# i2nico/MDAnalysis-MPI

Hardware: AMD Instinct MI355X
Metric: atom-frames/sec (RMSF) + achieved HBM GB/s fraction (higher is better)
Workload: dtype f64

## Files before the change

include/rmsf_hip.h:

```cpp
#ifndef RMSF_HIP_H
#define RMSF_HIP_H

#include <stddef.h>
#include <stdint.h>

#ifdef __cplusplus
extern "C" {
#endif

#define RMSF_ABI_VERSION 3

#define RMSF_OK 0
#define RMSF_EINVAL (-1)
#define RMSF_EHIP (-2)
#define RMSF_ENOMEM (-3)
#define RMSF_EEMPTY (-4)

#define RMSF_MODE_WELFORD 0
#define RMSF_MODE_SUM 1

#define RMSF_XFORM_DOUBLES 16
#define RMSF_MAX_SPLIT_FRAMES 4096
#define RMSF_PAIR_NEWTON 0
#define RMSF_PAIR_JACOBI 1
// ... 168 lines not shown
                                     double *d_ref, double *d_refinfo,
                                     void *stream);
int rmsf_reference_sums_sequential(int64_t n_sel, double mass_total,
                                   const double *d_ref, double *d_refinfo,
                                   void *stream);
int rmsf_superpose_sequential(const float *d_xyz, int64_t frame_stride,
                              int64_t n_frames, int64_t n_sel,
                              const int32_t *d_sel, const double *d_masses,
                              double mass_total, const double *d_ref,
                              const double *d_refinfo, double *d_xform,
                              void *stream);
int rmsf_frame_com_sequential(const float *d_xyz, int64_t frame_stride,
                              int64_t n_frames, int64_t n_sel,
                              const int32_t *d_sel, const double *d_masses,
                              double mass_total, double *d_xform, void *stream);
int rmsf_superpose_sequential_from_com(const float *d_xyz, int64_t frame_stride,
                                       int64_t n_frames, int64_t n_sel,
                                       const int32_t *d_sel, const double *d_ref,
                                       const double *d_refinfo, double *d_xform,
                                       void *stream);
int rmsf_inner_product_sequential(const float *d_xyz, int64_t frame_stride,
                                  int64_t n_frames, int64_t n_sel,
                                  const int32_t *d_sel, const double *d_ref,
                                  double *d_xform, void *stream);
int rmsf_superpose_sequential_qcp(int64_t n_frames, int64_t n_sel,
                                  const double *d_refinfo, double *d_xform,
                                  void *stream);
int rmsf_accumulate_sequential(const float *d_xyz, int64_t frame_stride,
                               int64_t n_frames, int64_t n_sel,
                               const int32_t *d_sel, const double *d_xform,
                               const double *d_refinfo, int mode, int64_t k0,
                               double *d_acc0, double *d_acc1, void *d_work,
                               size_t work_bytes, void *stream);

int rmsf_finalize(const double *d_m2, int64_t n_sel, int64_t n_frames,
                  double *d_rmsf, void *stream);

size_t rmsf_covariance_workspace_bytes(int64_t n_sel, int64_t n_frames);
int rmsf_covariance_accumulate(const float *d_xyz, int64_t frame_stride,
                               int64_t n_frames, int64_t n_sel,
                               const int32_t *d_sel, const double *d_xform,
                               const double *d_refinfo, const double *d_shift,
                               double *d_cov, int64_t ld, double *d_t1,
                               void *d_work, size_t work_bytes, void *stream);
int rmsf_covariance_finish(double *d_cov, int64_t ld, const double *d_t1,
                           int64_t n_coord, int64_t n_frames, void *stream);

size_t rmsf_pca_project_workspace_bytes(int64_t n_frames, int64_t n_sel,
                                        int64_t n_comp);
int rmsf_pca_project(const float *d_xyz, int64_t frame_stride,
                     int64_t n_frames, int64_t n_sel, const int32_t *d_sel,
                     const double *d_xform, const double *d_refinfo,
                     const double *d_mean, const double *d_comp, int64_t ldc,
                     int64_t n_comp, double *d_out, int64_t ldo, void *d_work,
                     size_t work_bytes, void *stream);

size_t rmsf_pca_backproject_workspace_bytes(int64_t n_frames, int64_t n_sel,
                                            int64_t n_cols);
int rmsf_pca_backproject(const float *d_xyz, int64_t frame_stride,
                         int64_t n_frames, int64_t n_sel, const int32_t *d_sel,
                         const double *d_xform, const double *d_refinfo,
                         const double *d_mean, const double *d_p, int64_t ldp,
                         int64_t n_cols, double *d_y, int64_t ldy,
                         int accumulate, void *d_work, size_t work_bytes,
                         void *stream);

// ... 234 lines not shown
```

mdanalysis-mpi_amd/csrc/rmsf_kernels.hip:

```cpp
#include <hip/hip_runtime.h>

#include <algorithm>
#include <cmath>
#include <cstdint>
#include <cstring>
#include <mutex>
#include <string>
#include <type_traits>
#include <unordered_map>
#include <vector>

#include "rmsf_hip.h"
#include "rmsf_device.h"

#define RMSF_EXPORT __attribute__((visibility("default")))
#ifndef RMSF_SHIFTED_SUMS
#define RMSF_SHIFTED_SUMS 1
#endif

namespace {

thread_local std::string g_err;

int fail(int code, const std::string &msg) {
// ... 291 lines not shown
  hdr[8] = p.S;
  hdr[9] = p.cw;
}

template <int U>
__global__ __launch_bounds__(kBlock) void k_welford_flat_sk(const float *__restrict__ xyz, int64_t stride4,
                                                            SkPlan pl, int64_t *__restrict__ hdr,
                                                            double *__restrict__ parts0,
                                                            double *__restrict__ parts1) {
  const int b = sk_range(pl, blockIdx.x);
  if (blockIdx.x == 0 && threadIdx.x == 0) sk_write_header(hdr, pl);
  int64_t lo = sk_lo(pl, b);
  const int64_t hi = sk_lo(pl, b + 1);
  int64_t slot = (int64_t)b * pl.P;
  while (lo < hi) {
    int64_t c, f0;
    const int len = (int)sk_seg_len(pl, lo, hi, &c, &f0);
    const int64_t i4 = c * kBlock + threadIdx.x;
    if (i4 < pl.lanes) {
      double m[4], q[4];
      wel_flat_run<U>(reinterpret_cast<const f32x4 *>(xyz) + f0 * stride4 + i4, stride4, len, m, q);
      const int64_t o = slot * (kBlock * 4) + 4 * threadIdx.x;
      store4(parts0 + o, parts1 + o, m, q);
    }
    lo += len;
    ++slot;
  }
}

struct SeqCoef {
  double c, r;
};

__global__ __launch_bounds__(kBlock) void k_seq_coef(int64_t k0, int64_t nf, SeqCoef *__restrict__ out) {
  const int64_t f = (int64_t)blockIdx.x * kBlock + threadIdx.x;
  if (f >= nf) return;
  const double k = (double)(k0 + f), k1 = k + 1.0;
  double r = __builtin_amdgcn_rcp(k1);
  double e = __builtin_fma(-k1, r, 1.0);
  r = __builtin_fma(r, e, r);
  e = __builtin_fma(-k1, r, 1.0);
  r = __builtin_fma(r, e, r);
  out[f] = SeqCoef{k / k1, r};
}

__device__ __forceinline__ double seq_div(double num, double k1, double r) {
  const double q0 = num * r;
  const double q = __builtin_fma(__builtin_fma(-k1, q0, num), r, q0);
  return (num == 0.0 || __builtin_isinf(num)) ? num : q;
}

template <int U, bool GATHER>
__global__ __launch_bounds__(kBlock) void k_welford_seq(const float *__restrict__ xyz, int64_t fstride, int64_t nf,
                                                        int64_t n_coord, const int32_t *__restrict__ sel,
                                                        int64_t k0, const SeqCoef *__restrict__ coef,
                                                        double *__restrict__ mean, double *__restrict__ ss) {
  const int64_t j = (int64_t)blockIdx.x * kBlock + threadIdx.x;
  if (j >= n_coord) return;
  double m = k0 > 0 ? mean[j] : 0.0, q = k0 > 0 ? ss[j] : 0.0;
  const float *__restrict__ p = xyz + (GATHER ? 3 * (int64_t)sel[j / 3] + j % 3 : j);
  auto step = [&](float v, const SeqCoef cf, double k, double k1) {
    const double x = (double)v;
    const double d = x - m;
    q = q + cf.c * (d * d);
    m = seq_div(k * m + x, k1, cf.r);
  };
  auto load = [&](float (&v)[U], SeqCoef (&c)[U], int64_t f) {
#pragma unroll
    for (int u = 0; u < U; ++u) {
      v[u] = __builtin_nontemporal_load(p + (f + u) * fstride);
      c[u] = coef[f + u];
    }
  };
  auto step_fast = [&](float v, const SeqCoef cf, double k, double k1) {
    const double x = (double)v;
    const double d = x - m;
// ... 440 lines not shown
                                                          int64_t n_sel, const int32_t *__restrict__ sel,
                                                          const double *__restrict__ ref, double *__restrict__ xform) {
  RMSF_SEQ_SLICE;
  const int64_t f = blockIdx.x;
  const int j = blockIdx.y;
  const float *__restrict__ fr = xyz + f * fstride;
  const double *t = xform + f * kXform;
  auto row = [&](int64_t a) -> int64_t { return 3 * (GATHER ? (int64_t)sel[a] : a); };
  double s;
  if (j < 9) {
    const int ax = j / 3, rb = j % 3;
    const double cx = t[9 + ax];
    s = RMSF_SEQ_SUM(
        n_sel, [&](int64_t a) { return SeqF1D{fr[row(a) + ax], ref[3 * a + rb]}; },
        [&](const SeqF1D &v, int64_t) { return ((double)v.x - cx) * v.d; });
  } else {
    const double c0 = t[9], c1 = t[10], c2 = t[11];
    s = RMSF_SEQ_SUM(
        n_sel,
        [&](int64_t a) {
          const float *p = fr + row(a);
          return SeqF3{p[0], p[1], p[2]};
        },
        [&](const SeqF3 &v, int64_t) {
          const double x1 = (double)v.x - c0, y1 = (double)v.y - c1, z1 = (double)v.z - c2;
          return x1 * x1 + y1 * y1 + z1 * z1;
        });
  }
  if (threadIdx.x == 0) xform[f * kXform + (j < 9 ? j : 13)] = s;
}
#undef RMSF_SEQ_SUM
#undef RMSF_SEQ_SLICE

__global__ __launch_bounds__(64) void k_seq_qcp(int64_t n_frames, int64_t n_sel, const double *__restrict__ refinfo,
                                                double *__restrict__ xform) {
  const int64_t f = (int64_t)blockIdx.x * 64 + threadIdx.x;
  if (f >= n_frames) return;
  double *t = xform + f * kXform;
  double A[9];
#pragma unroll
  for (int j = 0; j < 9; ++j) A[j] = t[j];
  const double E0 = (t[13] + refinfo[6]) * 0.5;
  double rot[9], rmsd;
  qcp_solve(A, E0, (double)n_sel, rot, &rmsd);
#pragma unroll
  for (int j = 0; j < 9; ++j) t[j] = rot[j];
  t[12] = rmsd;
  t[13] = t[14] = t[15] = 0.0;
}

template <int MODE, bool ALIGN, bool GATHER, int U>
__global__ __launch_bounds__(kBlock) void k_accum_seq(const float *__restrict__ xyz, int64_t fstride, int64_t nf,
                                                      int64_t n_sel, const int32_t *__restrict__ sel,
                                                      const double *__restrict__ xform,
                                                      const double *__restrict__ refinfo, int64_t k0,
                                                      const SeqCoef *__restrict__ coef, double *__restrict__ acc0,
                                                      double *__restrict__ acc1) {
  const int64_t a = (int64_t)blockIdx.x * kBlock + threadIdx.x;
  if (a >= n_sel) return;
  const double rc0 = ALIGN ? refinfo[0] : 0.0, rc1 = ALIGN ? refinfo[1] : 0.0, rc2 = ALIGN ? refinfo[2] : 0.0;
  double m[3], q[3] = {0.0, 0.0, 0.0};
#pragma unroll
  for (int c = 0; c < 3; ++c) {
    m[c] = k0 > 0 ? acc0[3 * a + c] : 0.0;
    if (MODE == RMSF_MODE_WELFORD && k0 > 0) q[c] = acc1[3 * a + c];
  }
  const float *__restrict__ p = xyz + 3 * (GATHER ? (int64_t)sel[a] : a);
  auto consume = [&](float x, float y, float z, int64_t f, double k) {
    if (ALIGN) apply_xform(x, y, z, xform + f * kXform, rc0, rc1, rc2);
    const float v[3] = {x, y, z};
    if (MODE == RMSF_MODE_SUM) {
#pragma unroll
      for (int c = 0; c < 3; ++c) m[c] = m[c] + (double)v[c];
    } else {
      const SeqCoef cf = coef[f];
#pragma unroll
      for (int c = 0; c < 3; ++c) {
        const double xx = (double)v[c];
        const double d = xx - m[c];
        q[c] = q[c] + cf.c * (d * d);
        m[c] = seq_div(k * m[c] + xx, k + 1.0, cf.r);
      }
    }
  };
  int64_t f = 0;
  double kb = (double)k0;
  for (; f + U <= nf; f += U) {
    float v[U][3];
#pragma unroll
    for (int u = 0; u < U; ++u) {
      const float *r = p + (f + u) * fstride;
#pragma unroll
      for (int c = 0; c < 3; ++c) v[u][c] = __builtin_nontemporal_load(r + c);
    }
#pragma unroll
    for (int u = 0; u < U; ++u, kb += 1.0) consume(v[u][0], v[u][1], v[u][2], f + u, kb);
  }
  for (; f < nf; ++f, kb += 1.0) {
    const float *r = p + f * fstride;
    consume(r[0], r[1], r[2], f, kb);
  }
#pragma unroll
  for (int c = 0; c < 3; ++c) {
    acc0[3 * a + c] = m[c];
    if (MODE == RMSF_MODE_WELFORD) acc1[3 * a + c] = q[c];
  }
}

template <int MODE, bool ALIGN, bool GATHER, int U, bool PLANES = false>
__global__ __launch_bounds__(kBlock) void k_accum_atoms_sk(const float *__restrict__ xyz, int64_t fstride,
                                                           const int32_t *__restrict__ sel,
                                                           const double *__restrict__ xform,
                                                           const double *__restrict__ refinfo, SkPlan pl,
                                                           int64_t *__restrict__ hdr, double *__restrict__ parts0,
                                                           double *__restrict__ parts1, int64_t ps = 0) {
  const int b = sk_range(pl, blockIdx.x);
  if (blockIdx.x == 0 && threadIdx.x == 0) sk_write_header(hdr, pl);
  const double rc0 = ALIGN ? refinfo[0] : 0.0, rc1 = ALIGN ? refinfo[1] : 0.0, rc2 = ALIGN ? refinfo[2] : 0.0;
  int64_t lo = uni64(sk_lo(pl, b));
  const int64_t hi = uni64(sk_lo(pl, b + 1));
  int64_t slot = (int64_t)b * pl.P;
  while (lo < hi) {
    int64_t c, f0;
    const int len = __builtin_amdgcn_readfirstlane((int)sk_seg_len(pl, lo, hi, &c, &f0));
    c = uni64(c);
    f0 = uni64(f0);
    const int64_t a = c * kBlock + threadIdx.x;
    if (a < pl.lanes) {
      const int64_t off = (PLANES ? 1 : 3) * (GATHER ? (int64_t)sel[a] : a);
      double m[3], q[3];
      accum_atoms_run<MODE, ALIGN, U, PLANES>(xyz + f0 * fstride + off, fstride, len,
                                              ALIGN ? xform + f0 * kXform : nullptr, rc0, rc1, rc2, m, q, ps);
      const int64_t o = slot * (kBlock * 3) + 3 * threadIdx.x;
      store3<MODE>(parts0 + o, parts1 + o, m, q);
    }
    lo += len;
    ++slot;
  }
}
// ... 2024 lines not shown
    if (d_sel) SEQIP(true, false);
    else SEQIP(false, false);
  }
#undef SEQIP
  return after_launch("k_seq_ip");
}

RMSF_EXPORT int rmsf_superpose_sequential_qcp(int64_t n_frames, int64_t n_sel, const double *d_refinfo,
                                              double *d_xform, void *stream) {
  if (!d_refinfo || !d_xform || n_sel < 1 || n_frames < 0)
    return fail(RMSF_EINVAL, "rmsf_superpose_sequential_qcp: bad arguments");
  if (n_frames == 0) return RMSF_OK;
  const unsigned fb = (unsigned)((n_frames + 63) / 64);
  hipLaunchKernelGGL(k_seq_qcp, dim3(fb), dim3(64), 0, S(stream), n_frames, n_sel, d_refinfo, d_xform);
  return after_launch("k_seq_qcp");
}

RMSF_EXPORT int rmsf_superpose_sequential_from_com(const float *d_xyz, int64_t fstride, int64_t n_frames,
                                                   int64_t n_sel, const int32_t *d_sel, const double *d_ref,
                                                   const double *d_refinfo, double *d_xform, void *stream) {
  if (!d_xyz || !d_ref || !d_refinfo || !d_xform || n_sel < 1 || n_frames < 0 || fstride < (d_sel ? 3 : 3 * n_sel))
    return fail(RMSF_EINVAL, "rmsf_superpose_sequential_from_com: bad arguments");
  if (int rc = rmsf_inner_product_sequential(d_xyz, fstride, n_frames, n_sel, d_sel, d_ref, d_xform, stream))
    return rc;
  return rmsf_superpose_sequential_qcp(n_frames, n_sel, d_refinfo, d_xform, stream);
}

RMSF_EXPORT int rmsf_superpose_sequential(const float *d_xyz, int64_t fstride, int64_t n_frames, int64_t n_sel,
                                          const int32_t *d_sel, const double *d_masses, double mass_total,
                                          const double *d_ref, const double *d_refinfo, double *d_xform,
                                          void *stream) {
  if (!d_xyz || !d_ref || !d_refinfo || !d_xform || n_sel < 1 || n_frames < 0 || fstride < (d_sel ? 3 : 3 * n_sel))
    return fail(RMSF_EINVAL, "rmsf_superpose_sequential: bad arguments");
  if (int rc = rmsf_frame_com_sequential(d_xyz, fstride, n_frames, n_sel, d_sel, d_masses, mass_total, d_xform,
                                         stream))
    return rc;
  return rmsf_superpose_sequential_from_com(d_xyz, fstride, n_frames, n_sel, d_sel, d_ref, d_refinfo, d_xform,
                                            stream);
}

RMSF_EXPORT int rmsf_accumulate_sequential(const float *d_xyz, int64_t fstride, int64_t n_frames, int64_t n_sel,
                                           const int32_t *d_sel, const double *d_xform, const double *d_refinfo,
                                           int mode, int64_t k0, double *d_acc0, double *d_acc1, void *d_work,
                                           size_t work_bytes, void *stream) {
  const bool wel = mode == RMSF_MODE_WELFORD;
  if ((mode != RMSF_MODE_WELFORD && mode != RMSF_MODE_SUM) || !d_xyz || !d_acc0 || (wel && (!d_acc1 || !d_work)) ||
      n_sel < 1 || n_frames < 0 || k0 < 0 || k0 + n_frames > (int64_t(1) << 53) ||
      fstride < (d_sel ? 3 : 3 * n_sel) || (d_xform != nullptr) != (d_refinfo != nullptr))
    return fail(RMSF_EINVAL, "rmsf_accumulate_sequential: bad arguments");
  if (n_frames == 0) return RMSF_OK;
  hipStream_t s = S(stream);
  const SeqCoef *coef = nullptr;
  if (wel) {
    if (work_bytes < rmsf_welford_sequential_workspace_bytes(n_frames))
      return fail(RMSF_EINVAL, "rmsf_accumulate_sequential: workspace too small");
    hipLaunchKernelGGL(k_seq_coef, dim3(grid1(n_frames)), dim3(kBlock), 0, s, k0, n_frames,
                       static_cast<SeqCoef *>(d_work));
    if (int rc = after_launch("k_seq_coef")) return rc;
    coef = static_cast<const SeqCoef *>(d_work);
  }
  const bool al = d_xform != nullptr, g = d_sel != nullptr;
  const dim3 grid((unsigned)grid1(n_sel));
#define SEQACC(MO, A, G)                                                                                    \
  hipLaunchKernelGGL((k_accum_seq<MO, A, G, 4>), grid, dim3(kBlock), 0, s, d_xyz, fstride, n_frames, n_sel, d_sel, \
                     d_xform, d_refinfo, k0, coef, d_acc0, d_acc1)
  auto launch = [&](auto MOc) {
    constexpr int MO = decltype(MOc)::value;
    if (al && g) SEQACC(MO, true, true);
    else if (al) SEQACC(MO, true, false);
    else if (g) SEQACC(MO, false, true);
    else SEQACC(MO, false, false);
  };
#undef SEQACC
  if (wel) launch(std::integral_constant<int, RMSF_MODE_WELFORD>{});
  else launch(std::integral_constant<int, RMSF_MODE_SUM>{});
  return after_launch("k_accum_seq");
}

RMSF_EXPORT int rmsf_finalize(const double *d_m2, int64_t n_sel, int64_t n_frames, double *d_rmsf, void *stream) {
  if (!d_m2 || !d_rmsf || n_sel < 1) return fail(RMSF_EINVAL, "rmsf_finalize: bad arguments");
  if (n_frames < 1) return fail(RMSF_EEMPTY, "rmsf_finalize: no frames");
  hipLaunchKernelGGL(k_finalize, dim3(grid1(n_sel)), dim3(kBlock), 0, S(stream), d_m2, n_sel, (double)n_frames,
                     d_rmsf);
  return after_launch("k_finalize");
}

RMSF_EXPORT int rmsf_qcp_batch(const double *d_A, const double *d_E0, const double *d_N, int64_t n, double *d_rot,
                               double *d_rmsd, void *stream) {
  if (!d_A || !d_E0 || !d_N || !d_rot || !d_rmsd || n < 0) return fail(RMSF_EINVAL, "rmsf_qcp_batch: bad arguments");
  if (n == 0) return RMSF_OK;
  hipLaunchKernelGGL(k_qcp_batch, dim3(grid1(n)), dim3(kBlock), 0, S(stream), d_A, d_E0, d_N, n, d_rot, d_rmsd);
  return after_launch("k_qcp_batch");
}

RMSF_EXPORT int rmsf_calc_rmsd_rotational_matrix(const double *h_ref, const double *h_conf, int64_t N, double *h_rot,
                                                 const double *h_weights, double *rmsd_out) {
  if (!h_ref || !h_conf || !h_rot || N < 1) return fail(RMSF_EINVAL, "CalcRMSDRotationalMatrix: bad arguments");
  const size_t cb = (size_t)N * 3 * sizeof(double);
  double *d = nullptr;
  const size_t total = 2 * cb + (size_t)N * sizeof(double) + 32 * sizeof(double);
  HIP_TRY(hipMalloc(&d, total));
  double *dref = d, *dconf = d + 3 * N, *dw = d + 6 * N, *dio = d + 7 * N;
  int rc = RMSF_OK;
  do {
    hipError_t e;
    if ((e = hipMemcpy(dref, h_ref, cb, hipMemcpyHostToDevice)) != hipSuccess) { rc = hip_fail("memcpy", e); break; }
    if ((e = hipMemcpy(dconf, h_conf, cb, hipMemcpyHostToDevice)) != hipSuccess) { rc = hip_fail("memcpy", e); break; }
    if (h_weights && (e = hipMemcpy(dw, h_weights, N * sizeof(double), hipMemcpyHostToDevice)) != hipSuccess) {
      rc = hip_fail("memcpy", e);
// ... 83 lines not shown
```

mdanalysis-mpi_amd/rmsf_amd/_lib.py:

```python
from __future__ import annotations

import ctypes
import os
from ctypes import POINTER, c_char_p, c_double, c_int, c_int32, c_int64, c_size_t, c_uint64, c_void_p

_HERE = os.path.dirname(os.path.abspath(__file__))
LIB_PATH = os.path.normpath(os.path.join(_HERE, "..", "lib", "librmsf_hip.so"))

RMSF_OK = 0
RMSF_EINVAL = -1
RMSF_EHIP = -2
RMSF_ENOMEM = -3
RMSF_EEMPTY = -4
RMSF_MODE_WELFORD = 0
RMSF_MODE_SUM = 1
RMSF_XFORM_DOUBLES = 16
RMSF_MAX_SPLIT_FRAMES = 4096
RMSF_REFINFO_DOUBLES = 2064
ABI_VERSION = 3
RMSF_PAIR_NEWTON = 0
RMSF_PAIR_JACOBI = 1
RMSF_PAIR_ZERO = 2


class RmsfError(RuntimeError):

    def __init__(self, code: int, func: str, msg: str):
        super().__init__(f"{func} failed with status {code}: {msg}")
        self.code = code


class RmsfEmptyError(RmsfError, ZeroDivisionError):
    """No frames to reduce.  Subclasses ZeroDivisionError because RMSF.py:39
    raises exactly that when two empty partials are merged."""


P = c_void_p
SIGNATURES = {
    "rmsf_abi_version": (c_int, []),
    "rmsf_last_error": (c_char_p, []),
    "rmsf_device_count": (c_int, [POINTER(c_int)]),
    "rmsf_set_device": (c_int, [c_int]),
    "rmsf_malloc": (c_int, [POINTER(c_void_p), c_size_t]),
    "rmsf_free": (c_int, [P]),
    "rmsf_memcpy_h2d": (c_int, [P, P, c_size_t, P]),
    "rmsf_memcpy_d2h": (c_int, [P, P, c_size_t, P]),
    "rmsf_memcpy2d_d2d": (c_int, [P, c_size_t, P, c_size_t, c_size_t, c_size_t, P]),
    "rmsf_stream_synchronize": (c_int, [P]),
# ... 2 lines not shown
    "rmsf_reference_setup_mean": (c_int, [P, c_double, c_int64, P, P, P, P, P]),
    "rmsf_fold_balanced_finalize": (c_int, [P, c_int64, c_int64, P, P, c_int64, P, P]),
    "rmsf_superpose_workspace_bytes": (c_size_t, [c_int64, c_int64]),
    "rmsf_superpose": (c_int, [P, c_int64, c_int64, c_int64, P, P, P, P, P, P, c_size_t, P]),
    "rmsf_superpose_planes": (c_int, [P, c_int64, c_int64, c_int64, c_int64, P, P, P, P, P, P, c_size_t, P]),
    "rmsf_superpose_compact": (c_int, [P, c_int64, c_int64, c_int64, P, P, P, P, P, P, c_size_t, P, c_int64, P]),
    "rmsf_accumulate_splits": (c_int, [c_int64, c_int64, c_int]),
    "rmsf_accumulate": (c_int, [P, c_int64, c_int64, c_int64, P, P, P, c_int, c_int, P, P, P]),
    "rmsf_split_count": (c_int64, [c_int64, c_int, c_int]),
    "rmsf_accumulate_balanced_workspace_bytes": (c_size_t, [c_int64, c_int64, c_int]),
    "rmsf_accumulate_balanced": (c_int, [P, c_int64, c_int64, c_int64, P, P, P, c_int, c_int, P, c_size_t, P]),
    "rmsf_fold_balanced": (c_int, [P, c_int64, c_int, c_int64, P, P, P]),
    "rmsf_accumulate_balanced_planes": (c_int, [P, c_int64, c_int64, c_int64, c_int64, P, P, P, c_int, c_int, P,
                                                c_size_t, P]),
    "rmsf_chan_merge": (c_int, [P, P, P, c_int, c_int64, P, P, P]),
    "rmsf_chan_reduce_steps": (c_int, [c_int, c_int, P, P, c_int]),
    "rmsf_chan_reduce": (c_int, [P, P, P, c_int, c_int64, c_int, P, P, P]),
    "rmsf_chan_merge_pair": (c_int, [P, P, c_int64, P, P, c_int64, c_int64, P]),
    "rmsf_sum_splits": (c_int, [P, c_int, c_int64, P, P]),
    "rmsf_divide": (c_int, [P, c_double, c_int64, P, P]),
    "rmsf_chan_weight": (c_int, [P, c_double, c_int64, P, P]),
    "rmsf_chan_deviation": (c_int, [P, P, P, c_double, c_int64, P, P]),
    "rmsf_finalize": (c_int, [P, c_int64, c_int64, P, P]),
    "rmsf_reference_setup_sequential": (c_int, [P, P, c_double, c_int64, P, P, c_double, P, P, P, P]),
    "rmsf_superpose_sequential": (c_int, [P, c_int64, c_int64, c_int64, P, P, c_double, P, P, P, P]),
    "rmsf_reference_centre_sequential": (c_int, [P, P, c_double, c_int64, P, P, c_double, P, P, P, P]),
    "rmsf_reference_sums_sequential": (c_int, [c_int64, c_double, P, P, P]),
    "rmsf_frame_com_sequential": (c_int, [P, c_int64, c_int64, c_int64, P, P, c_double, P, P]),
    "rmsf_inner_product_sequential": (c_int, [P, c_int64, c_int64, c_int64, P, P, P, P]),
    "rmsf_superpose_sequential_qcp": (c_int, [c_int64, c_int64, P, P, P]),
    "rmsf_superpose_sequential_from_com": (c_int, [P, c_int64, c_int64, c_int64, P, P, P, P, P]),
    "rmsf_accumulate_sequential": (c_int, [P, c_int64, c_int64, c_int64, P, P, P, c_int, c_int64, P, P, P, c_size_t,
                                           P]),
    "rmsf_welford_sequential_workspace_bytes": (c_size_t, [c_int64]),
    "rmsf_welford_sequential": (c_int, [P, c_int64, c_int64, c_int64, P, c_int64, P, P, P, c_size_t, P]),
    "rmsf_chan_shift_pack": (c_int, [P, P, P, c_int, P, c_double, c_int64, P, P]),
    "rmsf_fold_balanced_shift": (c_int, [P, c_int64, c_int64, P, P, P, c_int, P, P, P]),
    "rmsf_fold_balanced_shift_sliced": (c_int, [P, c_int64, c_int64, P, P, P, c_int, P, c_int64, P, P]),
    "rmsf_chan_shift_pack_sliced": (c_int, [P, P, P, c_int, P, c_double, c_int64, c_int64, P, P]),
    "rmsf_chan_shift_finish_slice": (c_int, [P, c_int64, P, c_int, P, c_int64, c_int64, P, P, P, P]),
    "rmsf_balanced_slab_chunks": (c_int, [P, c_int64, c_int64, c_int64, P]),
    "rmsf_accumulate_balanced_slab": (c_int, [P, c_int64, c_int64, c_int64, c_int64, c_int64, P, c_size_t, P]),
    "rmsf_fold_balanced_shift_slab": (c_int, [P, c_int64, c_int64, P, P, P, c_int, P, P, c_int64, c_int64, P]),
    "rmsf_chan_shift_finish": (c_int, [P, P, c_int, P, c_int64, c_int64, P, P, P, P]),
    "rmsf_covariance_workspace_bytes": (c_size_t, [c_int64, c_int64]),
    "rmsf_covariance_accumulate": (c_int, [P, c_int64, c_int64, c_int64, P, P, P, P, P, c_int64, P, P, c_size_t, P]),
    "rmsf_covariance_finish": (c_int, [P, c_int64, P, c_int64, c_int64, P]),
    "rmsf_pca_project_workspace_bytes": (c_size_t, [c_int64, c_int64, c_int64]),
    "rmsf_pca_project": (c_int, [P, c_int64, c_int64, c_int64, P, P, P, P, P, c_int64, c_int64, P, c_int64, P, c_size_t,
                                 P]),
    "rmsf_pca_backproject_workspace_bytes": (c_size_t, [c_int64, c_int64, c_int64]),
    "rmsf_pca_backproject": (c_int, [P, c_int64, c_int64, c_int64, P, P, P, P, P, c_int64, c_int64, P, c_int64, c_int,
                                     P, c_size_t, P]),
    "rmsf_symm_block_workspace_bytes": (c_size_t, [c_int64, c_int64]),
    "rmsf_symm_block": (c_int, [P, c_int64, c_int64, P, c_int64, c_int64, P, c_int64, P, c_size_t, P]),
    "rmsf_block_gram_workspace_bytes": (c_size_t, [c_int64, c_int64, c_int64]),
    "rmsf_block_gram": (c_int, [P, c_int64, c_int64, P, c_int64, c_int64, c_int64, P, c_int64, P, c_size_t, P]),
    "rmsf_block_update": (c_int, [c_double, P, c_int64, P, c_int64, c_int64, P, c_int64, c_int64, c_int64, P, c_int64,
                                  P]),
    "rmsf_pairwise_centres": (c_int,[P, c_int64, c_int64, c_int64, P, P, c_int, P, P, P]),
    "rmsf_pairwise_workspace_bytes": (c_size_t, [c_int64, c_int64]),
    "rmsf_pairwise_rmsd": (c_int, [P, c_int64, c_int64, c_int64, P, P, c_double, P, P, c_int, c_double, P, c_int64, P,
                                   c_size_t, P]),
    "rmsf_pairwise_centres_about": (c_int, [P, c_int64, c_int64, c_int64, P, P, P, P, P, P]),
    "rmsf_cross_workspace_bytes": (c_size_t, [c_int64, c_int64, c_int64]),
    "rmsf_cross_rmsd": (c_int, [P, c_int64, c_int64, P, P, P, P, c_int64, c_int64, P, P, P, c_int64, P, c_double,
# ... 152 lines not shown
```

mdanalysis-mpi_amd/rmsf_amd/engine.py:

```python
from __future__ import annotations

import ctypes

import numpy as np
import torch

from . import _lib
from ._lib import RMSF_MODE_SUM, RMSF_MODE_WELFORD, RMSF_REFINFO_DOUBLES, RMSF_XFORM_DOUBLES, call

F64 = torch.float64
F32 = torch.float32


def _ptr(t: torch.Tensor | None) -> int | None:
    return None if t is None else t.data_ptr()


class Engine:

    def __init__(self, device: torch.device | int | str | None = None):
        self.lib = _lib.load()
        if not torch.cuda.is_available():
            raise RuntimeError("rmsf_amd needs a HIP device (MI355X); none is visible -- no CPU fallback exists")
        if device is None:
            device = torch.device("cuda", torch.cuda.current_device())
        self.device = torch.device(device)
        if self.device.type != "cuda":
            raise ValueError(f"rmsf_amd runs on HIP devices only, got {self.device}")
        call("rmsf_set_device", self.device.index if self.device.index is not None else 0)

    @property
    def stream(self) -> int:
        return torch.cuda.current_stream(self.device).cuda_stream

    @property
    def side_stream(self) -> torch.cuda.Stream:
        if getattr(self, "_side", None) is None:
            self._side = torch.cuda.Stream(self.device)
        return self._side

    def empty(self, *shape, dtype=F64) -> torch.Tensor:
# ... 215 lines not shown
            call("rmsf_reference_setup_sequential", *args)
        else:
            call("rmsf_reference_centre_sequential", *args)
            after_centre()
            call("rmsf_reference_sums_sequential", n_sel, float(mass_total), ref.data_ptr(), info.data_ptr(),
                 self.stream)
        return avg, ref, info

    def superpose_seq(self, xyz_ptr: int, fstride: int, n_frames: int, n_sel: int, sel, masses,
                      mass_total: float, ref: torch.Tensor, refinfo: torch.Tensor, xform: torch.Tensor) -> None:
        call("rmsf_superpose_sequential", xyz_ptr, fstride, n_frames, n_sel, _ptr(sel), _ptr(masses),
             float(mass_total), ref.data_ptr(), refinfo.data_ptr(), xform.data_ptr(), self.stream)

    def frame_com_seq(self, xyz_ptr: int, fstride: int, n_frames: int, n_sel: int, sel, masses,
                      mass_total: float, xform: torch.Tensor) -> None:
        call("rmsf_frame_com_sequential", xyz_ptr, fstride, n_frames, n_sel, _ptr(sel), _ptr(masses),
             float(mass_total), xform.data_ptr(), self.stream)

    def superpose_seq_from_com(self, xyz_ptr: int, fstride: int, n_frames: int, n_sel: int, sel,
                               ref: torch.Tensor, refinfo: torch.Tensor, xform: torch.Tensor) -> None:
        call("rmsf_superpose_sequential_from_com", xyz_ptr, fstride, n_frames, n_sel, _ptr(sel), ref.data_ptr(),
             refinfo.data_ptr(), xform.data_ptr(), self.stream)

    def inner_product_seq(self, xyz_ptr: int, fstride: int, n_frames: int, n_sel: int, sel, ref: torch.Tensor,
                          xform: torch.Tensor) -> None:
        call("rmsf_inner_product_sequential", xyz_ptr, fstride, n_frames, n_sel, _ptr(sel), ref.data_ptr(),
             xform.data_ptr(), self.stream)

    def superpose_seq_qcp(self, n_frames: int, n_sel: int, refinfo: torch.Tensor, xform: torch.Tensor) -> None:
        call("rmsf_superpose_sequential_qcp", n_frames, n_sel, refinfo.data_ptr(), xform.data_ptr(), self.stream)

    def accumulate_seq(self, xyz_ptr: int, fstride: int, n_frames: int, n_sel: int, sel, xform, refinfo,
                       mode: int, k0: int, acc0: torch.Tensor, acc1: torch.Tensor | None,
                       work: torch.Tensor | None = None) -> torch.Tensor | None:
        if mode == RMSF_MODE_WELFORD:
            need = int(self.lib.rmsf_welford_sequential_workspace_bytes(n_frames))
            if work is None or work.numel() * work.element_size() < need:
                work = self.empty(max(need, 16) // 8)
        call("rmsf_accumulate_sequential", xyz_ptr, fstride, n_frames, n_sel, _ptr(sel), _ptr(xform),
             _ptr(refinfo), mode, k0, acc0.data_ptr(), _ptr(acc1), _ptr(work),
             0 if work is None else work.numel() * work.element_size(), self.stream)
        return work

    def finalize(self, m2: torch.Tensor, n_sel: int, n_frames: int, out: torch.Tensor) -> None:
        call("rmsf_finalize", m2.data_ptr(), n_sel, n_frames, out.data_ptr(), self.stream)

    def covariance_workspace_bytes(self, n_sel: int, n_frames: int) -> int:
        return int(self.lib.rmsf_covariance_workspace_bytes(n_sel, n_frames))

    def covariance_accumulate(self, xyz_ptr: int, fstride: int, n_frames: int, n_sel: int, sel, xform, refinfo,
                              shift: torch.Tensor, cov: torch.Tensor, t1: torch.Tensor,
                              work: torch.Tensor | None = None) -> None:
        n = 3 * n_sel
        if (cov.dtype != F64 or t1.dtype != F64 or shift.dtype != F64 or cov.dim() != 2 or cov.stride(1) != 1
                or cov.shape[0] < n or cov.shape[1] < n or t1.numel() < n or shift.numel() < n):
            raise ValueError("covariance_accumulate: buffer sizes")
        call("rmsf_covariance_accumulate", xyz_ptr, fstride, n_frames, n_sel, _ptr(sel), _ptr(xform), _ptr(refinfo),
             shift.data_ptr(), cov.data_ptr(), cov.stride(0), t1.data_ptr(), _ptr(work),
             0 if work is None else work.numel() * work.element_size(), self.stream)

    def covariance_finish(self, cov: torch.Tensor, t1: torch.Tensor, n_coord: int, n_frames: int) -> None:
        if cov.dim() != 2 or cov.stride(1) != 1 or cov.shape[0] < n_coord or cov.shape[1] < n_coord \
                or t1.numel() < n_coord:
            raise ValueError("covariance_finish: buffer sizes")
        call("rmsf_covariance_finish", cov.data_ptr(), cov.stride(0), t1.data_ptr(), n_coord, n_frames, self.stream)

    def pca_project_workspace_bytes(self, n_frames: int, n_sel: int, n_comp: int) -> int:
        return int(self.lib.rmsf_pca_project_workspace_bytes(n_frames, n_sel, n_comp))

    def pca_project(self, xyz_ptr: int, fstride: int, n_frames: int, n_sel: int, sel, xform, refinfo,
                    mean: torch.Tensor, comp: torch.Tensor, n_comp: int, out: torch.Tensor,
                    work: torch.Tensor | None = None) -> None:
        n = 3 * n_sel
        if (mean.dtype != F64 or comp.dtype != F64 or out.dtype != F64 or comp.dim() != 2 or out.dim() != 2
# ... 138 lines not shown
```

mdanalysis-mpi_amd/rmsf_amd/pipeline.py:

```python
from __future__ import annotations

import contextlib
import os
from collections import defaultdict
from dataclasses import dataclass, field

import numpy as np
import torch

from . import parallel
from ._lib import (RMSF_MAX_SPLIT_FRAMES, RMSF_MODE_SUM, RMSF_MODE_WELFORD, RMSF_REFINFO_DOUBLES, RMSF_XFORM_DOUBLES,
                   RmsfEmptyError)
from .engine import Engine
from .sources import Batch, DeviceSource, FrameList, _scattered

ALIGN_MODES = (None, "frame0", "average")


class KernelTimer:

    def __init__(self):
        self.spans = defaultdict(list)

    @contextlib.contextmanager
# ... 625 lines not shown
    m_dev, mass_total = None, float(n_sel)
    if masses is not None:
        m_np = masses.host if isinstance(masses, UploadedMasses) else np.ascontiguousarray(masses, dtype=np.float64)
        if m_np.size != n_sel:
            raise ValueError("masses must have one entry per selected atom")
        mass_total = float(m_np.sum())
        m_dev = masses.dev if isinstance(masses, UploadedMasses) else torch.as_tensor(m_np).to(eng.device)
    xf = eng.empty(max_batch, RMSF_XFORM_DOUBLES) if aligned else None
    rmsd = eng.empty(n_local) if (aligned and collect_rmsd) else None
    xf_last = eng.empty(n_local, RMSF_XFORM_DOUBLES) if (aligned and collect_transforms) else None
    xf_first = eng.empty(n_local, RMSF_XFORM_DOUBLES) if (collect_transforms and align == "average") else None

    from .sources import DeviceSource
    overlap = aligned and size == 1 and isinstance(source, DeviceSource) and n_sel >= EXACT_OVERLAP_MIN_ATOMS
    main = torch.cuda.current_stream(eng.device)
    side = None
    if overlap:
        side = getattr(eng, "_exact_side_stream", None)
        if side is None:
            side = eng._exact_side_stream = torch.cuda.Stream(eng.device)

    def on_side(fn):
        side.wait_stream(main)
        centred = torch.cuda.Event()
        with torch.cuda.stream(side):
            out = fn(lambda: centred.record(side))
        done = torch.cuda.Event()
        done.record(side)
        for t in out if isinstance(out, tuple) else (out,):
            if isinstance(t, torch.Tensor):
                t.record_stream(main)
        return out, (centred, done)

    def sweep(mode, acc0, acc1, ref=None, info=None, xf_out=None, pending=None, cov=None):
        work, k = None, 0
        for b in source.batches(frames, b0, b1, max_batch, eng.stream):
            if b.pstride:
                raise ValueError("exact=True reads (frame, atom, xyz) rows; this source handed over coordinate planes")
            x = None
            if aligned:
                x = xf[:b.n_frames]
                with _span(timer, "superpose", b.n_frames * n_sel):
                    if pending is None:
                        eng.superpose_seq(b.ptr, b.fstride, b.n_frames, n_sel, b.sel, m_dev, mass_total, ref, info,
                                          x)
                    else:
                        eng.frame_com_seq(b.ptr, b.fstride, b.n_frames, n_sel, b.sel, m_dev, mass_total, x)
                        main.wait_event(pending[0])
                        eng.inner_product_seq(b.ptr, b.fstride, b.n_frames, n_sel, b.sel, ref, x)
                        main.wait_event(pending[1])
                        pending = None
                        eng.superpose_seq_qcp(b.n_frames, n_sel, info, x)
                if rmsd is not None:
                    rmsd[k:k + b.n_frames].copy_(x[:, 12])
                if xf_out is not None:
                    xf_out[k:k + b.n_frames].copy_(x)
            with _span(timer, "accumulate", b.n_frames * n_sel):
                if aligned:
                    work = eng.accumulate_seq(b.ptr, b.fstride, b.n_frames, n_sel, b.sel, x, info, mode, k, acc0,
                                              acc1, work)
                else:
                    work = eng.welford_sequential(b.ptr, b.fstride, b.n_frames, n_sel, b.sel, k, acc0, acc1, work)
            if cov is not None:
                cov.add(b, x, info)
            k += b.n_frames
            b.done()

    ref = info = average = pending = None
    if aligned:
        def ref_frame_setup(after_centre=None):
            return reference_from_frame(eng, source, ref_frame, n_sel, m_dev, ref_owner, mass_total=mass_total,
                                        after_centre=after_centre)
        if overlap:
            (ref, info), pending = on_side(ref_frame_setup)
        else:
            ref, info = ref_frame_setup()
    if align == "average":
        total = eng.zeros(3 * n_sel)
        if n_local:
            sweep(RMSF_MODE_SUM, total, None, ref, info, xf_first, pending)
        elif pending is not None:
            main.wait_event(pending[1])
        pending = None
        parallel.allreduce_sum_ordered_(eng, total)

        def ref_avg_setup(after_centre=None):
            return eng.reference_setup_seq(n_sel, mass_total, total=total, n_frames=float(n_total), masses=m_dev,
                                           after_centre=after_centre)
        if overlap:
            (average, ref, info), pending = on_side(ref_avg_setup)
        else:
            average, ref, info = ref_avg_setup()
    mean, ss = eng.zeros(3 * n_sel), eng.zeros(3 * n_sel)
    covacc = comoment = None
    if covariance:
        if pending is not None:
            main.wait_event(pending[1])
        covacc = CovarianceAccumulator(eng, n_sel, max_batch,
                                       _covariance_shift(eng, source, frames, align, average, ref, info), timer)
    if n_local:
        sweep(RMSF_MODE_WELFORD, mean, ss, ref, info, xf_last, pending, covacc)
    elif pending is not None:
        main.wait_event(pending[1])
    if covacc is not None:
        comoment = covacc.finish(n_total, root)
    if size > 1:
        with _span(timer, "merge"):
            mean, ss = parallel.global_chan_exact(eng, mean, ss, [e - s for s, e in blocks], root, merge_order)
    rmsf = None
    if mean is not None:
        rmsf = eng.empty(n_sel)
        eng.finalize(ss, n_sel, n_total, rmsf)
    return PipelineResult(rmsf=rmsf, mean=None if mean is None else mean.view(n_sel, 3),
                          m2=None if ss is None else ss.view(n_sel, 3), n_frames=n_total, n_local=n_local,
                          block=(b0, b1), average=None if average is None else average.view(n_sel, 3), rmsd=rmsd,
                          transforms=xf_last, transforms_sweep1=xf_first,
                          extras={"exact": True, "merge_root": root, "merge_order": merge_order, "ref": ref,
                                  "refinfo": info}, comoment=comoment)


class UploadedMasses:

    def __init__(self, masses, device):
        self.host = np.ascontiguousarray(masses, dtype=np.float64)
        self.dev = torch.as_tensor(self.host).to(device)

    def __len__(self) -> int:
        return self.host.size


class CapturedPipeline:

    def __init__(self, eng: Engine, source, frames: FrameList, **kw):
        from .sources import DeviceSource

        if parallel.world()[1] > 1:
            raise NotImplementedError("graph capture is single-process (the RCCL merge is not captured)")
        if not isinstance(source, DeviceSource):
            raise TypeError("only HBM-resident (DeviceSource) pipelines can be captured")
        if kw.get("timer") is not None:
            raise ValueError("a KernelTimer cannot be captured")
        dev = eng.device
        if kw.get("masses") is not None and not isinstance(kw["masses"], UploadedMasses):
# ... 14 lines not shown
```

Measured before the change: 561.1 billion.

## Fuse per-frame superpose stages, compute Welford coefficients in LDS, fold finalize into accumulate

For small selections, one block per frame now computes the COM, the inner product and the QCP solve in a single kernel, replacing the separate COM/inner-product/QCP launches. The accumulate kernel computes Welford coefficients into shared memory instead of launching a separate coefficient kernel. On the last batch it writes RMSF directly, which removes the finalize launch. Accumulator buffers now use empty instead of zeros when frames exist. This cuts kernel launches and small memory passes, at the cost of a serial single-thread QCP step per block and extra LDS setup in every accumulate block.

```diff
diff --git a/include/rmsf_hip.h b/include/rmsf_hip.h
--- a/include/rmsf_hip.h
+++ b/include/rmsf_hip.h
@@ -224,6 +224,15 @@
                                const double *d_refinfo, int mode, int64_t k0,
                                double *d_acc0, double *d_acc1, void *d_work,
                                size_t work_bytes, void *stream);
+#define RMSF_SEQ_COEF_TABLE 1
+int rmsf_accumulate_sequential_finalize(const float *d_xyz, int64_t frame_stride,
+                                        int64_t n_frames, int64_t n_sel,
+                                        const int32_t *d_sel, const double *d_xform,
+                                        const double *d_refinfo, int mode,
+                                        int64_t k0, double *d_acc0, double *d_acc1,
+                                        void *d_work, size_t work_bytes, int flags,
+                                        int64_t n_total, double *d_rmsf,
+                                        void *stream);
 
 int rmsf_finalize(const double *d_m2, int64_t n_sel, int64_t n_frames,
                   double *d_rmsf, void *stream);
diff --git a/mdanalysis-mpi_amd/csrc/rmsf_kernels.hip b/mdanalysis-mpi_amd/csrc/rmsf_kernels.hip
--- a/mdanalysis-mpi_amd/csrc/rmsf_kernels.hip
+++ b/mdanalysis-mpi_amd/csrc/rmsf_kernels.hip
@@ -347,16 +347,20 @@
   double c, r;
 };
 
-__global__ __launch_bounds__(kBlock) void k_seq_coef(int64_t k0, int64_t nf, SeqCoef *__restrict__ out) {
-  const int64_t f = (int64_t)blockIdx.x * kBlock + threadIdx.x;
-  if (f >= nf) return;
-  const double k = (double)(k0 + f), k1 = k + 1.0;
+__device__ __forceinline__ SeqCoef seq_coef_at(int64_t kf) {
+  const double k = (double)kf, k1 = k + 1.0;
   double r = __builtin_amdgcn_rcp(k1);
   double e = __builtin_fma(-k1, r, 1.0);
   r = __builtin_fma(r, e, r);
   e = __builtin_fma(-k1, r, 1.0);
   r = __builtin_fma(r, e, r);
-  out[f] = SeqCoef{k / k1, r};
+  return SeqCoef{k / k1, r};
+}
+
+__global__ __launch_bounds__(kBlock) void k_seq_coef(int64_t k0, int64_t nf, SeqCoef *__restrict__ out) {
+  const int64_t f = (int64_t)blockIdx.x * kBlock + threadIdx.x;
+  if (f >= nf) return;
+  out[f] = seq_coef_at(k0 + f);
 }
 
 __device__ __forceinline__ double seq_div(double num, double k1, double r) {
@@ -863,30 +867,97 @@
 #undef RMSF_SEQ_SUM
 #undef RMSF_SEQ_SLICE
 
+__device__ __forceinline__ void seq_qcp_record(const double *a, double g1, double g2, int64_t n_sel, double *t) {
+  double A[9];
+#pragma unroll
+  for (int j = 0; j < 9; ++j) A[j] = a[j];
+  const double E0 = (g1 + g2) * 0.5;
+  double rot[9], rmsd;
+  qcp_solve(A, E0, (double)n_sel, rot, &rmsd);
+#pragma unroll
+  for (int j = 0; j < 9; ++j) t[j] = rot[j];
+  t[12] = rmsd;
+  t[13] = t[14] = t[15] = 0.0;
+}
+
 __global__ __launch_bounds__(64) void k_seq_qcp(int64_t n_frames, int64_t n_sel, const double *__restrict__ refinfo,
                                                 double *__restrict__ xform) {
   const int64_t f = (int64_t)blockIdx.x * 64 + threadIdx.x;
   if (f >= n_frames) return;
   double *t = xform + f * kXform;
-  double A[9];
-#pragma unroll
-  for (int j = 0; j < 9; ++j) A[j] = t[j];
-  const double E0 = (t[13] + refinfo[6]) * 0.5;
-  double rot[9], rmsd;
-  qcp_solve(A, E0, (double)n_sel, rot, &rmsd);
-#pragma unroll
-  for (int j = 0; j < 9; ++j) t[j] = rot[j];
-  t[12] = rmsd;
-  t[13] = t[14] = t[15] = 0.0;
-}
-
-template <int MODE, bool ALIGN, bool GATHER, int U>
+  seq_qcp_record(t, t[13], refinfo[6], n_sel, t);
+}
+
+constexpr int kSeqFrameWaves = 10;
+template <bool GATHER, bool MASSES>
+__global__ __launch_bounds__(64 * kSeqFrameWaves) void k_seq_frame(
+    const float *__restrict__ xyz, int64_t fstride, int64_t n_sel, const int32_t *__restrict__ sel,
+    const double *__restrict__ masses, double mass_total, const double *__restrict__ ref,
+    const double *__restrict__ refinfo, double *__restrict__ xform) {
+  __shared__ double slice[kSeqFrameWaves][kSeqBlk];
+  __shared__ double com[3];
+  __shared__ double sums[kSeqFrameWaves];
+  __builtin_assume(n_sel >= 1 && n_sel <= kSeqBlk);
+  const int64_t f = blockIdx.x;
+  const int w = __builtin_amdgcn_readfirstlane(threadIdx.x >> 6);
+  const bool lead = (threadIdx.x & 63) == 0;
+  const float *__restrict__ fr = xyz + f * fstride;
+  double *t = xform + f * kXform;
+  auto row = [&](int64_t a) -> int64_t { return 3 * (GATHER ? (int64_t)sel[a] : a); };
+  if (w < 3) {
+    const float *__restrict__ frc = fr + w;
+    const double s = wave_seq_sum(
+        n_sel, slice[w], [&](int64_t a) { return SeqF1D{frc[row(a)], MASSES ? masses[a] : 1.0}; },
+        [&](const SeqF1D &v, int64_t) { return (double)v.x * v.d; });
+    if (lead) t[9 + w] = com[w] = s / mass_total;
+  }
+  __syncthreads();
+  {
+    const int j = w;
+    double s;
+    if (j < 9) {
+      const int ax = j / 3, rb = j % 3;
+      const double cx = com[ax];
+      s = wave_seq_sum(
+          n_sel, slice[w], [&](int64_t a) { return SeqF1D{fr[row(a) + ax], ref[3 * a + rb]}; },
+          [&](const SeqF1D &v, int64_t) { return ((double)v.x - cx) * v.d; });
+    } else {
+      const double c0 = com[0], c1 = com[1], c2 = com[2];
+      s = wave_seq_sum(
+          n_sel, slice[w],
+          [&](int64_t a) {
+            const float *p = fr + row(a);
+            return SeqF3{p[0], p[1], p[2]};
+          },
+          [&](const SeqF3 &v, int64_t) {
+            const double x1 = (double)v.x - c0, y1 = (double)v.y - c1, z1 = (double)v.z - c2;
+            return x1 * x1 + y1 * y1 + z1 * z1;
+          });
+    }
+    if (lead) sums[j] = s;
+  }
+  __syncthreads();
+  if (threadIdx.x == 0) seq_qcp_record(sums, sums[9], refinfo[6], n_sel, t);
+}
+
+constexpr int kSeqCoefLds = 1024;
+template <int MODE, bool ALIGN, bool GATHER, int U, bool LCOEF>
 __global__ __launch_bounds__(kBlock) void k_accum_seq(const float *__restrict__ xyz, int64_t fstride, int64_t nf,
                                                       int64_t n_sel, const int32_t *__restrict__ sel,
                                                       const double *__restrict__ xform,
                                                       const double *__restrict__ refinfo, int64_t k0,
-                                                      const SeqCoef *__restrict__ coef, double *__restrict__ acc0,
-                                                      double *__restrict__ acc1) {
+                                                      const SeqCoef *__restrict__ gcoef, double *__restrict__ acc0,
+                                                      double *__restrict__ acc1, double nf_total,
+                                                      double *__restrict__ rmsf) {
+  __shared__ SeqCoef lcoef[LCOEF ? kSeqCoefLds : 1];
+  if (LCOEF) {
+    for (int f = threadIdx.x; f < (int)nf; f += kBlock) lcoef[f] = seq_coef_at(k0 + f);
+    __syncthreads();
+  }
+  auto coef = [&](int64_t f) -> SeqCoef {
+    if (LCOEF) return lcoef[f];
+    return gcoef[f];
+  };
   const int64_t a = (int64_t)blockIdx.x * kBlock + threadIdx.x;
   if (a >= n_sel) return;
   const double rc0 = ALIGN ? refinfo[0] : 0.0, rc1 = ALIGN ? refinfo[1] : 0.0, rc2 = ALIGN ? refinfo[2] : 0.0;
@@ -904,7 +975,7 @@
 #pragma unroll
       for (int c = 0; c < 3; ++c) m[c] = m[c] + (double)v[c];
     } else {
-      const SeqCoef cf = coef[f];
+      const SeqCoef cf = coef(f);
 #pragma unroll
       for (int c = 0; c < 3; ++c) {
         const double xx = (double)v[c];
@@ -936,6 +1007,7 @@
     acc0[3 * a + c] = m[c];
     if (MODE == RMSF_MODE_WELFORD) acc1[3 * a + c] = q[c];
   }
+  if (MODE == RMSF_MODE_WELFORD && rmsf) rmsf[a] = sqrt((q[0] + q[1] + q[2]) / nf_total);
 }
 
 template <int MODE, bool ALIGN, bool GATHER, int U, bool PLANES = false>
@@ -3026,6 +3098,19 @@
                                           void *stream) {
   if (!d_xyz || !d_ref || !d_refinfo || !d_xform || n_sel < 1 || n_frames < 0 || fstride < (d_sel ? 3 : 3 * n_sel))
     return fail(RMSF_EINVAL, "rmsf_superpose_sequential: bad arguments");
+  if (n_sel <= kSeqBlk) {
+    if (n_frames == 0) return RMSF_OK;
+    const bool g = d_sel != nullptr, m = d_masses != nullptr;
+#define SEQFRAME(G, M)                                                                                          \
+  hipLaunchKernelGGL((k_seq_frame<G, M>), dim3((unsigned)n_frames), dim3(64 * kSeqFrameWaves), 0, S(stream), d_xyz, \
+                     fstride, n_sel, d_sel, d_masses, mass_total, d_ref, d_refinfo, d_xform)
+    if (g && m) SEQFRAME(true, true);
+    else if (g) SEQFRAME(true, false);
+    else if (m) SEQFRAME(false, true);
+    else SEQFRAME(false, false);
+#undef SEQFRAME
+    return after_launch("k_seq_frame");
+  }
   if (int rc = rmsf_frame_com_sequential(d_xyz, fstride, n_frames, n_sel, d_sel, d_masses, mass_total, d_xform,
                                          stream))
     return rc;
@@ -3033,42 +3118,58 @@
                                             stream);
 }
 
+RMSF_EXPORT int rmsf_accumulate_sequential_finalize(const float *d_xyz, int64_t fstride, int64_t n_frames,
+                                                    int64_t n_sel, const int32_t *d_sel, const double *d_xform,
+                                                    const double *d_refinfo, int mode, int64_t k0, double *d_acc0,
+                                                    double *d_acc1, void *d_work, size_t work_bytes, int flags,
+                                                    int64_t n_total, double *d_rmsf, void *stream) {
+  const bool wel = mode == RMSF_MODE_WELFORD;
+  if ((mode != RMSF_MODE_WELFORD && mode != RMSF_MODE_SUM) || !d_xyz || !d_acc0 || (wel && (!d_acc1 || !d_work)) ||
+      n_sel < 1 || n_frames < 0 || k0 < 0 || k0 + n_frames > (int64_t(1) << 53) ||
+      fstride < (d_sel ? 3 : 3 * n_sel) || (d_xform != nullptr) != (d_refinfo != nullptr) ||
+      (flags & ~RMSF_SEQ_COEF_TABLE) || (d_rmsf && (!wel || n_frames < 1 || n_total < k0 + n_frames)))
+    return fail(RMSF_EINVAL, "rmsf_accumulate_sequential: bad arguments");
+  if (n_frames == 0) return RMSF_OK;
+  hipStream_t s = S(stream);
+  const SeqCoef *coef = nullptr;
+  const bool lcoef = wel && n_frames <= kSeqCoefLds && !(flags & RMSF_SEQ_COEF_TABLE);
+  if (wel) {
+    if (work_bytes < rmsf_welford_sequential_workspace_bytes(n_frames))
+      return fail(RMSF_EINVAL, "rmsf_accumulate_sequential: workspace too small");
+    if (!lcoef) {
+      hipLaunchKernelGGL(k_seq_coef, dim3(grid1(n_frames)), dim3(kBlock), 0, s, k0, n_frames,
+                         static_cast<SeqCoef *>(d_work));
+      if (int rc = after_launch("k_seq_coef")) return rc;
+    }
+    coef = static_cast<const SeqCoef *>(d_work);
+  }
+  const bool al = d_xform != nullptr, g = d_sel != nullptr;
+  const dim3 grid((unsigned)grid1(n_sel));
+  const double nf_total = (double)n_total;
+#define SEQACC(MO, A, G, L)                                                                                    \
+  hipLaunchKernelGGL((k_accum_seq<MO, A, G, 4, L>), grid, dim3(kBlock), 0, s, d_xyz, fstride, n_frames, n_sel, \
+                     d_sel, d_xform, d_refinfo, k0, coef, d_acc0, d_acc1, nf_total, d_rmsf)
+  auto launch = [&](auto MOc, auto Lc) {
+    constexpr int MO = decltype(MOc)::value;
+    constexpr bool L = decltype(Lc)::value;
+    if (al && g) SEQACC(MO, true, true, L);
+    else if (al) SEQACC(MO, true, false, L);
+    else if (g) SEQACC(MO, false, true, L);
+    else SEQACC(MO, false, false, L);
+  };
+#undef SEQACC
+  if (lcoef) launch(std::integral_constant<int, RMSF_MODE_WELFORD>{}, std::true_type{});
+  else if (wel) launch(std::integral_constant<int, RMSF_MODE_WELFORD>{}, std::false_type{});
+  else launch(std::integral_constant<int, RMSF_MODE_SUM>{}, std::false_type{});
+  return after_launch("k_accum_seq");
+}
+
 RMSF_EXPORT int rmsf_accumulate_sequential(const float *d_xyz, int64_t fstride, int64_t n_frames, int64_t n_sel,
                                            const int32_t *d_sel, const double *d_xform, const double *d_refinfo,
                                            int mode, int64_t k0, double *d_acc0, double *d_acc1, void *d_work,
                                            size_t work_bytes, void *stream) {
-  const bool wel = mode == RMSF_MODE_WELFORD;
-  if ((mode != RMSF_MODE_WELFORD && mode != RMSF_MODE_SUM) || !d_xyz || !d_acc0 || (wel && (!d_acc1 || !d_work)) ||
-      n_sel < 1 || n_frames < 0 || k0 < 0 || k0 + n_frames > (int64_t(1) << 53) ||
-      fstride < (d_sel ? 3 : 3 * n_sel) || (d_xform != nullptr) != (d_refinfo != nullptr))
-    return fail(RMSF_EINVAL, "rmsf_accumulate_sequential: bad arguments");
-  if (n_frames == 0) return RMSF_OK;
-  hipStream_t s = S(stream);
-  const SeqCoef *coef = nullptr;
-  if (wel) {
-    if (work_bytes < rmsf_welford_sequential_workspace_bytes(n_frames))
-      return fail(RMSF_EINVAL, "rmsf_accumulate_sequential: workspace too small");
-    hipLaunchKernelGGL(k_seq_coef, dim3(grid1(n_frames)), dim3(kBlock), 0, s, k0, n_frames,
-                       static_cast<SeqCoef *>(d_work));
-    if (int rc = after_launch("k_seq_coef")) return rc;
-    coef = static_cast<const SeqCoef *>(d_work);
-  }
-  const bool al = d_xform != nullptr, g = d_sel != nullptr;
-  const dim3 grid((unsigned)grid1(n_sel));
-#define SEQACC(MO, A, G)                                                                                    \
-  hipLaunchKernelGGL((k_accum_seq<MO, A, G, 4>), grid, dim3(kBlock), 0, s, d_xyz, fstride, n_frames, n_sel, d_sel, \
-                     d_xform, d_refinfo, k0, coef, d_acc0, d_acc1)
-  auto launch = [&](auto MOc) {
-    constexpr int MO = decltype(MOc)::value;
-    if (al && g) SEQACC(MO, true, true);
-    else if (al) SEQACC(MO, true, false);
-    else if (g) SEQACC(MO, false, true);
-    else SEQACC(MO, false, false);
-  };
-#undef SEQACC
-  if (wel) launch(std::integral_constant<int, RMSF_MODE_WELFORD>{});
-  else launch(std::integral_constant<int, RMSF_MODE_SUM>{});
-  return after_launch("k_accum_seq");
+  return rmsf_accumulate_sequential_finalize(d_xyz, fstride, n_frames, n_sel, d_sel, d_xform, d_refinfo, mode, k0,
+                                             d_acc0, d_acc1, d_work, work_bytes, 0, 0, nullptr, stream);
 }
 
 RMSF_EXPORT int rmsf_finalize(const double *d_m2, int64_t n_sel, int64_t n_frames, double *d_rmsf, void *stream) {
diff --git a/mdanalysis-mpi_amd/rmsf_amd/_lib.py b/mdanalysis-mpi_amd/rmsf_amd/_lib.py
--- a/mdanalysis-mpi_amd/rmsf_amd/_lib.py
+++ b/mdanalysis-mpi_amd/rmsf_amd/_lib.py
@@ -14,6 +14,7 @@
 RMSF_EEMPTY = -4
 RMSF_MODE_WELFORD = 0
 RMSF_MODE_SUM = 1
+RMSF_SEQ_COEF_TABLE = 1
 RMSF_XFORM_DOUBLES = 16
 RMSF_MAX_SPLIT_FRAMES = 4096
 RMSF_REFINFO_DOUBLES = 2064
@@ -82,6 +83,8 @@
     "rmsf_superpose_sequential_from_com": (c_int, [P, c_int64, c_int64, c_int64, P, P, P, P, P]),
     "rmsf_accumulate_sequential": (c_int, [P, c_int64, c_int64, c_int64, P, P, P, c_int, c_int64, P, P, P, c_size_t,
                                            P]),
+    "rmsf_accumulate_sequential_finalize": (c_int, [P, c_int64, c_int64, c_int64, P, P, P, c_int, c_int64, P, P, P,
+                                                    c_size_t, c_int, c_int64, P, P]),
     "rmsf_welford_sequential_workspace_bytes": (c_size_t, [c_int64]),
     "rmsf_welford_sequential": (c_int, [P, c_int64, c_int64, c_int64, P, c_int64, P, P, P, c_size_t, P]),
     "rmsf_chan_shift_pack": (c_int, [P, P, P, c_int, P, c_double, c_int64, P, P]),
diff --git a/mdanalysis-mpi_amd/rmsf_amd/engine.py b/mdanalysis-mpi_amd/rmsf_amd/engine.py
--- a/mdanalysis-mpi_amd/rmsf_amd/engine.py
+++ b/mdanalysis-mpi_amd/rmsf_amd/engine.py
@@ -6,7 +6,8 @@
 import torch
 
 from . import _lib
-from ._lib import RMSF_MODE_SUM, RMSF_MODE_WELFORD, RMSF_REFINFO_DOUBLES, RMSF_XFORM_DOUBLES, call
+from ._lib import (RMSF_MODE_SUM, RMSF_MODE_WELFORD, RMSF_REFINFO_DOUBLES, RMSF_SEQ_COEF_TABLE, RMSF_XFORM_DOUBLES,
+                   call)
 
 F64 = torch.float64
 F32 = torch.float32
@@ -288,14 +289,16 @@
 
     def accumulate_seq(self, xyz_ptr: int, fstride: int, n_frames: int, n_sel: int, sel, xform, refinfo,
                        mode: int, k0: int, acc0: torch.Tensor, acc1: torch.Tensor | None,
-                       work: torch.Tensor | None = None) -> torch.Tensor | None:
+                       work: torch.Tensor | None = None, *, rmsf: torch.Tensor | None = None, n_total: int = 0,
+                       coef_table: bool = False) -> torch.Tensor | None:
         if mode == RMSF_MODE_WELFORD:
             need = int(self.lib.rmsf_welford_sequential_workspace_bytes(n_frames))
             if work is None or work.numel() * work.element_size() < need:
                 work = self.empty(max(need, 16) // 8)
-        call("rmsf_accumulate_sequential", xyz_ptr, fstride, n_frames, n_sel, _ptr(sel), _ptr(xform),
+        call("rmsf_accumulate_sequential_finalize", xyz_ptr, fstride, n_frames, n_sel, _ptr(sel), _ptr(xform),
              _ptr(refinfo), mode, k0, acc0.data_ptr(), _ptr(acc1), _ptr(work),
-             0 if work is None else work.numel() * work.element_size(), self.stream)
+             0 if work is None else work.numel() * work.element_size(), RMSF_SEQ_COEF_TABLE if coef_table else 0,
+             n_total, _ptr(rmsf), self.stream)
         return work
 
     def finalize(self, m2: torch.Tensor, n_sel: int, n_frames: int, out: torch.Tensor) -> None:
diff --git a/mdanalysis-mpi_amd/rmsf_amd/pipeline.py b/mdanalysis-mpi_amd/rmsf_amd/pipeline.py
--- a/mdanalysis-mpi_amd/rmsf_amd/pipeline.py
+++ b/mdanalysis-mpi_amd/rmsf_amd/pipeline.py
@@ -681,7 +681,7 @@
                 t.record_stream(main)
         return out, (centred, done)
 
-    def sweep(mode, acc0, acc1, ref=None, info=None, xf_out=None, pending=None, cov=None):
+    def sweep(mode, acc0, acc1, ref=None, info=None, xf_out=None, pending=None, cov=None, fin=None):
         work, k = None, 0
         for b in source.batches(frames, b0, b1, max_batch, eng.stream):
             if b.pstride:
@@ -706,8 +706,9 @@
                     xf_out[k:k + b.n_frames].copy_(x)
             with _span(timer, "accumulate", b.n_frames * n_sel):
                 if aligned:
+                    last = fin is not None and k + b.n_frames == n_local
                     work = eng.accumulate_seq(b.ptr, b.fstride, b.n_frames, n_sel, b.sel, x, info, mode, k, acc0,
-                                              acc1, work)
+                                              acc1, work, rmsf=fin if last else None, n_total=n_total)
                 else:
                     work = eng.welford_sequential(b.ptr, b.fstride, b.n_frames, n_sel, b.sel, k, acc0, acc1, work)
             if cov is not None:
@@ -725,7 +726,7 @@
         else:
             ref, info = ref_frame_setup()
     if align == "average":
-        total = eng.zeros(3 * n_sel)
+        total = (eng.empty if n_local else eng.zeros)(3 * n_sel)
         if n_local:
             sweep(RMSF_MODE_SUM, total, None, ref, info, xf_first, pending)
         elif pending is not None:
@@ -740,7 +741,9 @@
             (average, ref, info), pending = on_side(ref_avg_setup)
         else:
             average, ref, info = ref_avg_setup()
-    mean, ss = eng.zeros(3 * n_sel), eng.zeros(3 * n_sel)
+    new = eng.empty if n_local else eng.zeros
+    mean, ss = new(3 * n_sel), new(3 * n_sel)
+    fin = eng.empty(n_sel) if (aligned and size == 1 and n_local) else None
     covacc = comoment = None
     if covariance:
         if pending is not None:
@@ -748,7 +751,7 @@
         covacc = CovarianceAccumulator(eng, n_sel, max_batch,
                                        _covariance_shift(eng, source, frames, align, average, ref, info), timer)
     if n_local:
-        sweep(RMSF_MODE_WELFORD, mean, ss, ref, info, xf_last, pending, covacc)
+        sweep(RMSF_MODE_WELFORD, mean, ss, ref, info, xf_last, pending, covacc, fin)
     elif pending is not None:
         main.wait_event(pending[1])
     if covacc is not None:
@@ -756,8 +759,8 @@
     if size > 1:
         with _span(timer, "merge"):
             mean, ss = parallel.global_chan_exact(eng, mean, ss, [e - s for s, e in blocks], root, merge_order)
-    rmsf = None
-    if mean is not None:
+    rmsf = fin
+    if mean is not None and rmsf is None:
         rmsf = eng.empty(n_sel)
         eng.finalize(ss, n_sel, n_total, rmsf)
     return PipelineResult(rmsf=rmsf, mean=None if mean is None else mean.view(n_sel, 3),
```

New measurement: 561.1 billion (median of 3 runs). No clear change (-0.0%).
